# yuguangnudt/VEC_VAD

Hardware: AMD Instinct MI355X
Metric: spatio-temporal cubes/sec (train step) (higher is better)
Workload: dtype f32

## Files before the change

### vec_vad_amd/bank.py

```python
import ctypes as C
import math
import os
from collections import OrderedDict
from types import SimpleNamespace

import torch

from . import _lib as L

RAW_C, OF_C = 3, 2
HW0 = 32


def _ceil(a, b):
    return (a + b - 1) // b * b


def _pick_ksplit(groups, ntiles, ncu=256, epilogue=1.5, max_wg=1024):
    best, best_cost = 1, None
    for ks in range(1, ntiles + 1):
        if groups * ks > max_wg and ks > 1:
            break
        rounds = -(-groups * ks // ncu)
        cost = rounds * (-(-ntiles // ks) + epilogue)
        if best_cost is None or cost < best_cost - 1e-9:
            best, best_cost = ks, cost
    return best


class UnitSpec:

    def __init__(self, role, erase, tgt):
        self.role, self.erase, self.tgt = role, erase, tgt
        self.out_c = RAW_C if role == 'raw' else OF_C


class ConvLayer:
    def __init__(self, idx, H, cin, cout, mode, src, skip=None, up=None):
        self.idx, self.H, self.cin, self.cout, self.mode, self.src, self.skip, self.up = idx, H, cin, cout, mode, src, skip, up
        self.cinp = _ceil(cin, 16)


class BankLayout:

    def __init__(self, nf, in_ch):
        self.nf, self.in_ch = nf, in_ch
        c = nf
        Ls = [ConvLayer(0, 32, in_ch, nf, L.IN_CUBE, 'cube'), ConvLayer(1, 32, nf, nf, L.IN_ACT, 0)]
        H = 32
        for d in range(3):
            H //= 2
            Ls.append(ConvLayer(len(Ls), H, c, 2 * c, L.IN_POOL, len(Ls) - 1))
            Ls.append(ConvLayer(len(Ls), H, 2 * c, 2 * c, L.IN_ACT, len(Ls) - 1))
            c *= 2
        self.convT = []
        skips = [5, 3, 1]
        for u in range(3):
            self.convT.append((len(Ls) - 1, H, c, c // 2))
            H *= 2
            Ls.append(ConvLayer(len(Ls), H, c, c // 2, L.IN_CAT, None, skip=skips[u], up=u))
            Ls.append(ConvLayer(len(Ls), H, c // 2, c // 2, L.IN_ACT, len(Ls) - 1))
            c //= 2
        self.convs = Ls
        off = 0
        self.p = OrderedDict()
        for l in Ls:
            self.p['c%d.w' % l.idx] = (off, (l.cout, l.cin, 3, 3)); off += _ceil(l.cout * l.cin * 9, 4)
            self.p['c%d.b' % l.idx] = (off, (l.cout,)); off += l.cout
            self.p['c%d.g' % l.idx] = (off, (l.cout,)); off += l.cout
            self.p['c%d.beta' % l.idx] = (off, (l.cout,)); off += l.cout
        for u, (_, _, ci, co) in enumerate(self.convT):
            self.p['t%d.w' % u] = (off, (ci, co, 3, 3)); off += ci * co * 9
            self.p['t%d.b' % u] = (off, (co,)); off += co
        self.p['o.w'] = (off, (4, nf, 1, 1)); off += 4 * nf
        self.p['o.b'] = (off, (4,)); off += 4
        self.U = _ceil(off, 4)
        off = 0
        self.b = OrderedDict()
        for l in Ls:
            self.b['c%d.rm' % l.idx] = (off, (l.cout,)); off += l.cout
            self.b['c%d.rv' % l.idx] = (off, (l.cout,)); off += l.cout
        self.UB = _ceil(off, 4)
        off = 0
        self.pk = OrderedDict()
        for l in Ls:
            self.pk['c%d.f' % l.idx] = (off, 0, l.cin, l.cinp, l.cout, 'c%d.w' % l.idx); off += 9 * l.cinp * l.cout
            if l.idx > 0:
                self.pk['c%d.d' % l.idx] = (off, 1, l.cout, l.cout, l.cin, 'c%d.w' % l.idx); off += 9 * l.cout * l.cin
        for u, (_, _, ci, co) in enumerate(self.convT):
            self.pk['t%d.f' % u] = (off, 2, ci, ci, co, 't%d.w' % u); off += 9 * ci * co
            self.pk['t%d.d' % u] = (off, 3, co, co, ci, 't%d.w' % u); off += 9 * ci * co
        self.pkw = OrderedDict()
        for l in Ls:
            self.pkw['c%d.f' % l.idx] = (off, 0, l.cin, l.cinp, l.cout, 'c%d.w' % l.idx); off += 16 * l.cinp * l.cout
# ... 41 lines not shown
        for fn, args, label in self.calls:
            rc = fn(*args, stream)
            if rc:
                L.check(rc, label)


class UNetBank:
    def __init__(self, units, nf=32, tot_raw_num=5, tot_of_num=1, padding=False, active=None, device='cuda',
                 lambda_raw=1.0, lambda_of=1.0):
        self.lib = L.lib()
        self.ncu = int(self.lib.vv_num_cus())
        self.units = list(units)
        self.G = len(self.units)
        self.nf, self.tot_raw, self.tot_of, self.padding = nf, tot_raw_num, tot_of_num, padding
        if nf % 32:
            raise L.VecVadHipError('features_root must be a multiple of 32 for the MFMA tiles (got %d)' % nf)
        if nf not in (32, 64):
            raise L.VecVadHipError('features_root = %d: nf = 32 (the value of every shipped config.cfg) and nf = 64 (the default of '
                                   'SelfCompleteNet1raw1of, model/unet.py:563) are implemented -- the fused 1x1 output conv + loss '
                                   'kernels are instantiated for these two widths' % nf)
        self.in_ch = RAW_C * (tot_raw_num if padding else tot_raw_num - 1)
        self.lay = BankLayout(nf, self.in_ch)
        self.g0, self.Ga = active if active is not None else (0, self.G)
        self.lambda_raw, self.lambda_of = lambda_raw, lambda_of
        self.device = torch.device(device)
        self._alloc_state()
        self.ws = {}

    @property
    def adam_t(self):
        return self._adam_t

    @adam_t.setter
    def adam_t(self, t):
        self._adam_t = int(t)
        self._adam_t_dev.fill_(int(t))

    def _alloc_state(self):
        d, lay, G = self.device, self.lay, self.G
        nconv = len(lay.convs)

        def switch(name):
            v = os.environ.get(name, '1')
            if v not in ('0', '1'):
                raise ValueError('%s must be 0 or 1, got %r' % (name, v))
            return v == '1'

        def launch_set(name, default, words, names):
            v = os.environ.get(name, default).lower()
            if v.startswith('set:'):
                picked = frozenset(t for t in v[4:].split(',') if t)
                if not picked <= names:
                    raise ValueError('%s=%s: unknown entries %s' % (name, v, sorted(picked - names)))
                return picked
            if v not in words:
                raise ValueError('%s must be one of %s or set:..., got %r' % (name, ' / '.join(words), v))
            return '0' if v == 'off' else v

        self.precision = os.environ.get('VV_PRECISION', 'fp32').lower()
        if self.precision not in ('fp32', 'bf16'):
            raise ValueError("VV_PRECISION / [mi355x] precision must be 'fp32' or 'bf16', got %r" % self.precision)
        if self.nf != 32 and self.precision != 'fp32':
            raise L.VecVadHipError('mixed precision is implemented for features_root = 32 only')
        self.cflag = L.CONV_BF16 if self.precision == 'bf16' else 0
        self.dz16 = switch('VV_BF16_DZ') and bool(self.cflag)
        self.da16 = switch('VV_BF16_DA') and bool(self.cflag)
        self.y16 = switch('VV_BF16_Y') and self.dz16 and self.da16
        self.split_dcat = switch('VV_SPLIT_DCAT') and self.da16
        self.fflag = self.cflag | ((L.CONV_OUT_BF16 | L.CONV_ALLSRC_BF16) if self.y16 else 0)
        self.fuse_outconv = switch('VV_FUSE_OUTCONV')
        wino_env = switch('VV_WINOGRAD')
        self.wino = wino_env and not self.cflag
        self.wino_wgrad = switch('VV_WINOGRAD_WGRAD') and wino_env
        self.wgrad_flag = 256
        w44_words = ('0', 'off', '1', 'dgrad', 'all')
        w44_names = frozenset(['f%d' % i for i in range(nconv)] + ['d%d' % i for i in range(1, nconv)])
        self.w44_mode = launch_set('VV_WINO44', 'dgrad', w44_words, w44_names)
        self._w44_tables = {}
        self._w44_eval_used = set()
        self.w44_eval_mode = launch_set('VV_WINO44_EVAL', '1', w44_words, w44_names)
        self.fuse_bn_sums = switch('VV_FUSE_BN_SUMS')
        self.fuse_bn_sums_t = switch('VV_FUSE_BN_SUMS_T')
        fold = launch_set('VV_FUSE_BN_APPLY', '1', ('0', 'off', '1'), frozenset(str(i) for i in range(nconv)))
        self.fold_bn_apply = frozenset(int(t) for t in fold) if isinstance(fold, frozenset) else \
            frozenset() if fold == '0' else frozenset((0, 2, 4))
        self.group_reduce = switch('VV_GROUP_REDUCE')
        self.eval_fold = switch('VV_EVAL_FOLD') and not self.cflag

        self.params = torch.zeros(G, lay.U, device=d)
        self.bufs = torch.zeros(G, lay.UB, device=d)
        self.gb = [0, lay.p['c4.w'][0], lay.p['c8.w'][0], lay.U]
        self._gb_c = (C.c_int64 * len(self.gb))(*self.gb)
        self.grads = torch.zeros(G * lay.U, device=d)
        self.adam_m = None
        self.adam_v = None
        self._adam_t = 0
        self._adam_t_dev = torch.zeros(1, dtype=torch.long, device=d)
        self._adam_sc = torch.zeros(2, device=d)
        self.nbt = torch.zeros(G, len(lay.convs), dtype=torch.long, device=d)
        self.packed = torch.zeros(G, lay.UP, device=d)
        cin_p = lay.convs[0].cinp
        chmap = torch.full((G, cin_p), -1, dtype=torch.int32)
        oc = torch.zeros(G, dtype=torch.int32)
        tsrc = torch.zeros(G, dtype=torch.int32)
        tcoff = torch.zeros(G, dtype=torch.int32)
        for g, u in enumerate(self.units):
            if self.padding:
                for k in range(self.in_ch):
                    chmap[g, k] = -1 if u.erase * RAW_C <= k < (u.erase + 1) * RAW_C else k
            else:
                for k in range(self.in_ch):
                    chmap[g, k] = k if k < u.erase * RAW_C else k + RAW_C
            oc[g] = u.out_c
            tsrc[g] = 0 if u.role == 'raw' else 1
            tcoff[g] = u.tgt * (RAW_C if u.role == 'raw' else OF_C)
        self.chmap, self.oc, self.tsrc, self.tcoff = chmap.to(d), oc.to(d), tsrc.to(d), tcoff.to(d)
        direct = [(k, v) for k, v in lay.pk.items() if not (self.wino and k[0] == 'c')]
        ents = (L.PackEntry * len(direct))()
        mx = 0
        for i, (k, (off, mode, K, KP, N, src)) in enumerate(direct):
            ents[i] = L.PackEntry(lay.p[src][0], off, mode | (L.PACK_BF16 if self.cflag else 0), K, KP, N)
            mx = max(mx, 9 * KP * N)
        self.pack_table = torch.frombuffer(bytearray(bytes(ents)), dtype=torch.uint8).to(d)
        self.pack_n, self.pack_max = len(direct), mx
        head = lambda k: k[0] == 'c' and int(k[1:k.index('.')]) <= 1
        self.pack_head_n = sum(1 for k, _ in direct if head(k))
        assert all(head(k) for k, _ in direct[:self.pack_head_n])
        wents = (L.PackEntry * len(lay.pkw))()
        wmx = 0
        for i, (k, (off, mode, K, KP, N, src)) in enumerate(lay.pkw.items()):
            wents[i] = L.PackEntry(lay.p[src][0], off, mode, K, KP, N)
            wmx = max(wmx, KP * N)
        self.pack_table_w = torch.frombuffer(bytearray(bytes(wents)), dtype=torch.uint8).to(d)
        self.pack_w_n, self.pack_w_max = len(lay.pkw), wmx
        self.pack_w_head_n = sum(1 for k in lay.pkw if head(k))
        assert all(head(k) for k in list(lay.pkw)[:self.pack_w_head_n])
        self.eval_path = ('BatchNorm folded into filter + bias once per model state (vv_fold_bn), ReLU in the conv epilogue, plain loads'
                          if self.eval_fold else 'train-mode kernel family with running statistics')
        self.params_eval = self.packed_eval = None
        self._eval_key = None
        self._state_ver = 0
        fents = (L.FoldEntry * len(lay.convs))()
        for i, l in enumerate(lay.convs):
            fents[i] = L.FoldEntry(lay.p['c%d.w' % l.idx][0], lay.p['c%d.b' % l.idx][0], lay.p['c%d.g' % l.idx][0],
                                   lay.p['c%d.beta' % l.idx][0], lay.b['c%d.rm' % l.idx][0], lay.b['c%d.rv' % l.idx][0],
                                   l.cout, l.cin * 9)
        self.fold_table = torch.frombuffer(bytearray(bytes(fents)), dtype=torch.uint8).to(d)
        self.ab_ident = torch.stack([torch.ones(G, lay.cmax), torch.zeros(G, lay.cmax)]).to(d)

    def to(self, device):
        device = torch.device(device)
        if device == self.device:
            return self
        for n in ('params', 'bufs', 'grads', '_adam_t_dev', '_adam_sc', 'nbt', 'packed', 'chmap', 'oc', 'tsrc', 'tcoff', 'pack_table', 'pack_table_w', 'fold_table', 'ab_ident'):
            setattr(self, n, getattr(self, n).to(device))
        self._w44_tables, self._w44_eval_table = {}, None
        if self.adam_m is not None:
            self.adam_m, self.adam_v = self.adam_m.to(device), self.adam_v.to(device)
        self.device = device
        self.ws = {}
        self.params_eval = self.packed_eval = None
        self._eval_key = None
        return self

    def param_view(self, g, key):
        off, shape = self.lay.p[key]
        n = 1
        for s in shape:
# ... 377 lines not shown
        nf = self.nf
        f = lambda *s: torch.empty(*s, device=d, dtype=torch.float32)
        P = _Plan()
        pbase, kbase = self._p(self.params, g0 * U), self._p(self.packed, g0 * UP)
        abg = lay.cmax
        HWp = HW0 * HW0
        last = lay.convs[-1]
        self._alloc_outconv_bwd(ws, B)
        ws.D = {l.idx: f(Ga, B * l.H * l.H, l.cin) for l in lay.convs if l.idx > 0}

        def dcat_views(m):
            dcat = ws.D[m.idx]
            skipc = lay.convs[m.skip].cout
            if self.split_dcat and 2 * skipc == m.cin and skipc & (skipc - 1) == 0:
                plane = B * m.H * m.H * skipc * 2
                return (L.view(dcat, skipc, 0, dcat.stride(0)), L.view(dcat.data_ptr() + plane, skipc, 0, dcat.stride(0)), skipc)
            return (L.view(dcat, m.cin, 0, dcat.stride(0)), L.View(dcat.data_ptr(), dcat.stride(0), m.cin, skipc), 0)
        ws.DT = [f(Ga, B * H * H, ci) for (_, H, ci, co) in lay.convT]
        ws.dz2 = [f(Ga, B * HWp * nf), f(Ga, B * HWp * nf)]
        ws.dz = ws.dz2[0]
        ws.bnscr = f(Ga, 2 * lay.cmax)
        ws.bscr = f(Ga, (B * HWp + 1023) // 1024 * lay.cmax)
        ws.dstats = f(Ga, max(max(lib.vv_conv_ntiles2(B, l.H, l.H, L.CONV3, self.cflag), lib.vv_conv_ntiles(B, l.H, l.H),
                                  lib.vv_wino_ntiles(B, l.H)) * 2 * l.cin for l in lay.convs if l.mode == L.IN_CAT))

        t_of = {sidx: u for u, (sidx, _, _, _) in enumerate(lay.convT)}
        skip_of = {m.skip: m for m in lay.convs if m.mode == L.IN_CAT}
        pool_of = {m.src: m for m in lay.convs if m.mode == L.IN_POOL}
        act_of = {m.src: m for m in lay.convs if m.mode == L.IN_ACT}

        def dA_for(i):
            if i == last.idx:
                return L.view(ws.gA_last, nf, 0, ws.gA_last.stride(0)), None, 0
            if i in t_of:
                t = ws.DT[t_of[i]]
                return L.view(t, t.shape[2], 0, t.stride(0)), None, 0
            if i in skip_of:
                dp = ws.D[pool_of[i].idx] if i in pool_of else None
                return dcat_views(skip_of[i])[0], dp.data_ptr() if dp is not None else None, dp.stride(0) if dp is not None else 0
            dn = ws.D[i + 1]
            return L.view(dn, lay.convs[i + 1].cin, 0, dn.stride(0)), None, 0

        def wgrad(kind, H, cinp, cout, bf16_flags, wide):
            tiles = ((cinp + 31) // 32) * (cout // 32)
            nt = lib.vv_wgrad_ntiles(kind, B, H, H)
            ks = _pick_ksplit(Ga * tiles, nt, ncu=3 * self.ncu, max_wg=12 * self.ncu) if wide else \
                _pick_ksplit(Ga * tiles, nt, ncu=self.ncu, max_wg=4 * self.ncu)
            w = SimpleNamespace(bf16=False, ks=ks, kw=0)
            ntb, nblk, kw = C.c_int32(), C.c_int32(), C.c_int32()
            if self.cflag and lib.vv_wgrad_bf16_plan(kind | (bf16_flags << 8), B, H, H, cinp, cout,
                                                     C.byref(ntb), C.byref(nblk), C.byref(kw)):
                w = SimpleNamespace(bf16=True, ks=self._ks_bf16(Ga * nblk.value, ntb.value), kw=kw.value)
            w.nslab = w.ks * max(w.kw, 1)
            w.size = tiles * w.nslab * 9 * 1024
            return w

        rec = []
        for l in lay.convs:
            r = wgrad(L.CONV3, l.H, l.cinp, l.cout, (L.WGRAD_DY_BF16 | L.WGRAD_X_BF16) if self.y16 else 0,
                      self.wino_wgrad and not self.cflag)
            r.dA, r.dpool, r.dpg = dA_for(l.idx)
            r.dz16 = self.dz16 and r.bf16
            r.dflags = (self.cflag | ((L.CONV_ALLSRC_BF16 if self.y16 else L.CONV_SRC_BF16) if r.dz16 else 0) |
                        (L.CONV_OUT_BF16 if self.da16 else 0))
            r.dgrad = self._route(B, l, True, r.dflags) if l.idx > 0 else None
            r.partials, r.bn_sums_of = 0, None
            rec.append(r)
        trec = [wgrad(L.CONVT_FWD, H, ci, co, 0, False) for (_, H, ci, co) in lay.convT]
        for t in trec:
            t.bn_sums_of = None

        rec[last.idx].partials = L.BNBWD_PARTIALS_PER_CUBE
        for l in lay.convs:
            r, j = rec[l.idx], l.idx - 1
            if self.fuse_bn_sums and l.mode == L.IN_ACT and l.idx > 0 and l.src == j and j not in t_of and j not in skip_of \
                    and j not in pool_of and (self.wino or (self.y16 and r.bf16 and l.H == 32 and l.cin % 64 != 0)):
                r.bn_sums_of, rec[j].partials = j, r.dgrad[3]
        for u, (sidx, _, _, _) in enumerate(lay.convT):
            if self.fuse_bn_sums and self.fuse_bn_sums_t and not self.cflag and sidx != last.idx and sidx not in skip_of \
                    and sidx not in pool_of and sidx not in act_of:
                trec[u].bn_sums_of, rec[sidx].partials = sidx, L.BNBWD_PARTIALS_PER_TTILE

        for l, r in zip(lay.convs, rec):
            r.fold = (self.wino and self.wino_wgrad and l.idx in self.fold_bn_apply and l.idx != last.idx and l.cout <= 256
                      and r.dpool is None and (l.idx == 0 or (l.H in (16, 8) and r.dgrad[0] is not lib.vv_conv_wino44)))

        wtot = 0
        for w in rec + trec:
            w.woff, wtot = wtot, wtot + w.size
        ws.wpart = f(Ga, wtot)
        ws.bntab = {i: f(Ga, L.BNBWD_TAB_ROWS * lay.convs[i].cout) for i, r in enumerate(rec) if r.fold}
        wpg = ws.wpart.stride(0)
        pending = []

        def reduce_wgrad(key, kind, cin, cinp, cout, w, label, bucket_done, **kw_):
            gptr, gstride = self._g(key + '.w')
            if not self.group_reduce:
                P.add(lib.vv_wgrad_reduce, (kind, Ga, cin, cinp, cout, w.nslab, ws.wpart.data_ptr() + 4 * w.woff, wpg, gptr, gstride),
                      label, stream=1, **kw_)
                return
            pending.append((kind, cin, cinp, cout, w, gptr, gstride))
            if not bucket_done:
                return
            ents = (L.ReduceEntry * len(pending))()
            start = 0
            for n, (kind, cin, cinp, cout, w, gptr, gstride) in enumerate(pending):
                ents[n] = L.ReduceEntry(kind, cin, cout, cout // 32, w.nslab, start, w.woff, (gptr - self.grads.data_ptr()) // 4, gstride)
                start += ((cinp + 31) // 32) * (cout // 32) * 36
            tab = torch.frombuffer(bytearray(bytes(ents)), dtype=torch.uint8).to(d)
            P.keep.append(tab)
            P.add(lib.vv_wgrad_reduce_grouped, (tab.data_ptr(), len(pending), start, Ga, ws.wpart.data_ptr(), wpg, self.grads.data_ptr()),
                  label, stream=1, **kw_)
            del pending[:]

        def bn_sums(cp, j):
            yj = ws.y[j]
            cp.bn_z, cp.bn_z_gstride = yj.data_ptr(), yj.stride(0)
            cp.bn_a, cp.bn_b = self._p(ws.ab[0, j]), self._p(ws.ab[1, j])
            cp.bn_mean, cp.bn_invstd = self._p(ws.ab[2, j]), self._p(ws.ab[3, j])
            cp.bn_gstride, cp.bn_partial = abg, ws.bnpart.data_ptr()

        y = ws.y[last.idx]
        P.add(lib.vv_outconv_bwd, (Ga, B, HWp, nf, ws.dout4.data_ptr(), y.data_ptr(), y.stride(0), self._p(ws.ab[0, last.idx]),
                                   self._p(ws.ab[1, last.idx]), abg, pbase + 4 * lay.p['o.w'][0], U, ws.gA_last.data_ptr(),
                                   ws.gA_last.stride(0), ws.ocpart.data_ptr(),
                                   self._p(ws.ab[2, last.idx]), self._p(ws.ab[3, last.idx]), ws.bnpart.data_ptr(),
                                   (1 if self.da16 else 0) | (2 if self.y16 else 0)), 'outconv_bwd')
        assert self._g('o.w')[1] == self._g('o.b')[1]
        P.add(lib.vv_outconv_bwd_reduce, (Ga, nf, B, ws.ocpart.data_ptr(), self._p(self.oc, g0), self._g('o.w')[0],
                                          self._g('o.b')[0], self._g('o.w')[1]), 'outconv_bwd_reduce')

        order = [l.idx for l in reversed(lay.convs)]

        def conv_bwd(l):
            i, r = l.idx, rec[l.idx]
            y = ws.y[i]
            pos = order.index(i)
            dzb = ws.dz2[pos % 2]
            reuse_wait = ('wdone%d' % order[pos - 2],) if pos >= 2 and not r.fold else ()
            bp = L.BnBwdParams(Ga, B, l.H, l.H, l.cout,
                               (L.BNBWD_DZ_BF16 if r.dz16 else 0) | r.partials | (L.BNBWD_DA_BF16 if self.da16 else 0) |
                               (L.BNBWD_Y_BF16 if self.y16 else 0), y.data_ptr(), y.stride(0), self._p(ws.ab[0, i]), self._p(ws.ab[1, i]),
                               self._p(ws.ab[2, i]), self._p(ws.ab[3, i]), abg, r.dA, r.dpool, r.dpg, dzb.data_ptr(), dzb.stride(0),
                               ws.bnpart.data_ptr())
            P.keep.append(bp)
            if not r.partials:
                P.add(lib.vv_bn_bwd_reduce, (C.byref(bp),), 'bn_bwd_reduce%d' % i, wait=reuse_wait)
            if r.fold:
                tab = ws.bntab[i]
                P.add(lib.vv_bn_bwd_sums, (C.byref(bp), pbase + 4 * lay.p['c%d.g' % i][0], U, self._g('c%d.g' % i)[0],
                                           self._g('c%d.beta' % i)[0], self._g('c%d.g' % i)[1], tab.data_ptr(), tab.stride(0)),
                      'bn_bwd_sum%d' % i, record='dy%d' % i)
            else:
                P.add(lib.vv_bn_bwd_apply, (C.byref(bp), pbase + 4 * lay.p['c%d.g' % i][0], U, self._g('c%d.g' % i)[0],
                                            self._g('c%d.beta' % i)[0], self._g('c%d.g' % i)[1], ws.bnscr.data_ptr()), 'bn_bwd_apply%d' % i,
                      record='dy%d' % i, wait=reuse_wait if r.partials else ())
            if i > 0:
                Dl = ws.D[i]
                fn, panel = r.dgrad[:2]
                cp = L.ConvParams(L.CONV3, L.IN_PLAIN, Ga, B, l.H, l.H, l.cout, l.cout, l.cin,
                                  L.View(dzb.data_ptr(), dzb.stride(0), l.cout, 0), None, None, 0, L.NULL_VIEW, 0, r.dflags, None,
                                  kbase + 4 * panel, UP, None, 0, L.view(Dl, l.cin, 0, Dl.stride(0)),
                                  ws.dstats.data_ptr() if l.mode == L.IN_CAT else None)
                if r.fold:
                    cp.in_mode, cp.src0, cp.src1 = L.IN_BNBWD, r.dA, L.view(y, l.cout, 0, y.stride(0))
                    cp.a, cp.ab_gstride = ws.bntab[i].data_ptr(), ws.bntab[i].stride(0)
                if l.mode == L.IN_CAT:
                    v0, v1, osplit = dcat_views(l)
# ... 200 lines not shown
```

### vec_vad_amd/csrc/vv_wino44.hip

```cpp
#include <type_traits>
#include "vv_common.h"
namespace {

constexpr int W4N = 384;
constexpr int W4G = 2;
constexpr int W4T = 32;
constexpr int SB4_MASK = 0x386;
constexpr float PA = 0.75f, PB = 1.5f;
constexpr float PA2 = PA * PA, PB2 = PB * PB, PA3 = PA2 * PA, PB3 = PB2 * PB;
constexpr float PA2B2 = PA2 * PB2, PS2 = PA2 + PB2, PAB2 = PA * PB2, PA2B = PA2 * PB;

__device__ __forceinline__ void vv_lds_barrier4() {
  asm volatile("s_waitcnt lgkmcnt(0)" ::: "memory");
  __builtin_amdgcn_s_barrier();
  asm volatile("" ::: "memory");
}

template <int H_>
struct W4Geo {
  static constexpr int TPI = H_ / 4;
  static constexpr int TP = TPI * TPI;
  static constexpr int TPW = TP < W4T ? TP : W4T;
  static constexpr int NI = W4T / TPW;
  static constexpr int PARTS = TP / TPW;
  static constexpr int TROWS = TPW / TPI;
  static constexpr int HH = 4 * TROWS + 2, HW = H_ + 2;
  static constexpr int HWQ = (HW + 3) / 4;
  static constexpr int ROW = H_ == 32 ? 38 : (H_ == 16 ? 21 : (H_ == 8 ? 14 : 8));
  static constexpr int IMG = H_ == 32 ? HH * ROW : (H_ == 16 ? 400 : (H_ == 8 ? 146 : 49));
  static constexpr int PLANE = NI * IMG;
  static constexpr int tile_slot(const int l) {
    const int tim = l / TPW, rem = l % TPW;
    return tim * IMG + 4 * (rem / TPI) * ROW + rem % TPI;
  }
  static constexpr bool ok() {
    if (ROW < 4 * HWQ || IMG < HH * ROW) return false;
    for (int l0 = 0; l0 < 32; l0 += 16) {
      unsigned seen = 0;
      for (int l = l0; l < l0 + 16; ++l) {
        const unsigned bit = 1u << (tile_slot(l) & 15);
        if (seen & bit) return false;
        seen |= bit;
      }
    }
    return true;
  }
};
static_assert(W4Geo<32>::ok() && W4Geo<16>::ok() && W4Geo<8>::ok() && W4Geo<4>::ok(), "LDS image: bank conflicts or overlap");

template <int H_, bool NS>
__global__ void __launch_bounds__(W4N * W4G, 3)
wino44_conv_kernel(const vv_conv_params p, const int NT, const int NN, const int total, const int nper) {
  using G_ = W4Geo<H_>;
  constexpr int TPI = G_::TPI, TPW = G_::TPW, NI = G_::NI, PARTS = G_::PARTS, HH = G_::HH, HW = G_::HW, HWQ = G_::HWQ;
  constexpr int ROW = G_::ROW, IMG = G_::IMG, PLANE = G_::PLANE;
  constexpr int CK = 8, Q = 2;
  constexpr int HY0 = PARTS == 1 ? 1 : 0, HR = PARTS == 1 ? HH - 2 : HH;
  constexpr int NITEMS = NI * HR * H_ * Q;
  constexpr int STN = NS ? W4N * W4G : W4N;
  constexpr int NIT = (NITEMS + STN - 1) / STN;
  constexpr int HALO8 = 4 * PLANE;
  constexpr int EX8 = 6 * 8 * 64 * 2;
  constexpr int L8 = HALO8 > EX8 ? HALO8 : EX8;
  __shared__ v2f lds_all[W4G][L8 + 6 * 32 + 256];
  const int wv = __builtin_amdgcn_readfirstlane((int)(threadIdx.x >> 6));
  const int sg = wv / 6;
  v2f* const lds8 = lds_all[sg];
  float* lds = reinterpret_cast<float*>(lds8);
  v2f* const halo = NS ? lds_all[0] : lds8;

  int w = vv_xcd_remap(blockIdx.x, nper);
  if (w >= total) return;
  int nn, pt, g;
  bool live = true;
  if constexpr (NS) {
    const int NNW = NN / W4G;
    nn = (w % NNW) * W4G + sg; w /= NNW;
    pt = w % NT;
    g = w / NT;
  } else {
    nn = w % NN; w /= NN;
    const int NTP = (NT + W4G - 1) / W4G;
    const int pt_ = (w % NTP) * W4G + sg;
    live = pt_ < NT;
    pt = live ? pt_ : NT - 1;
    g = w / NTP;
  }

  const int tid = threadIdx.x - sg * W4N, lane = tid & 63, half = lane >> 5, l31 = lane & 31;
  const int stid = NS ? (int)threadIdx.x : tid;
  const int xi = wv - sg * 6;
  const int img0 = (pt / PARTS) * NI, part = pt % PARTS;
  const int y0 = part * (4 * G_::TROWS) - 1;
  const VVSrc s = vv_make_src(p, g, H_, H_);
  const int Cout = p.Cout, CinP = p.CinP, KQ = CinP >> 3;
  const int co0 = nn * 32;
  const float* __restrict__ wg = p.w + (int64_t)g * p.w_gstride;

  unsigned valid = 0;
  unsigned itm[NIT];
  const int tile = (img0 * H_ + y0) * H_ - 1;
  const int q4 = (stid % Q) * 4;
  for (int hp = stid; hp < NI * HH * HW; hp += STN) {
    const int hx = hp % HW, t = hp / HW;
    const int hy = t % HH, im = t / HH;
    if (hx == 0 || hx == HW - 1 || hy < HY0 || hy >= HY0 + HR) {
      const int sl = im * IMG + hy * ROW + (hx & 3) * HWQ + (hx >> 2);
#pragma unroll
      for (int pl = 0; pl < 4; ++pl) halo[pl * PLANE + sl] = (v2f){0.f, 0.f};
    }
  }
#pragma unroll
  for (int k = 0; k < NIT; ++k) {
    const int it = stid + k * STN;
    const int q = it % Q, hp = it / Q;
    const int hx = hp % H_ + 1, t = hp / H_;
    const int hy = t % HR + HY0, im = t / HR;
    const bool inr = NITEMS % STN == 0 || it < NITEMS;
    const int y = y0 + hy;
    const bool ok = inr && (unsigned)y < (unsigned)H_ && (img0 + im) < s.B;
    valid |= ok ? (1u << k) : 0u;
    const int pixv = (im * H_ + hy) * H_ + hx;
    const int sl = inr ? q * 2 * PLANE + im * IMG + hy * ROW + (hx & 3) * HWQ + (hx >> 2) : 0xFFFF;
    itm[k] = ((unsigned)sl << 16) | (unsigned)pixv;
  }
  static_assert((NI * H_ + HH) * H_ + HW < 65536 && 4 * PLANE < 65535, "packed item word");
  const __amdgpu_buffer_rsrc_t rsW = __builtin_amdgcn_make_buffer_rsrc(const_cast<float*>(wg), 0, 0x7FFFFFFF, 0x00020000);
  const unsigned bvo = (unsigned)(half * Cout + co0 + l31) * 8u;
  const int bsub = 2 * Cout * 8;
  const int bnu = KQ * 2 * bsub;
  const int bxi = xi * 6 * bnu;
  const int nact = s.mode == VV_IN_ACT ? CinP : (s.mode == VV_IN_CAT ? s.csplit : 0);
  float4* const ab4 = reinterpret_cast<float4*>((NS ? lds_all[0] : lds8) + L8 + 6 * 32);
  for (int i = stid; i < (nact >> 2); i += STN) {
    ab4[i] = *reinterpret_cast<const float4*>(s.a + 4 * i);
    ab4[(CinP >> 2) + i] = *reinterpret_cast<const float4*>(s.b + 4 * i);
  }
  float4 r[NIT];
  auto issue = [&](const int c0) {
    const bool second = __builtin_amdgcn_readfirstlane((int)((s.mode == VV_IN_CAT) && c0 >= s.csplit)) != 0;
    const float* base = second ? s.p1 + s.co1 : s.p0 + s.co0;
    const int cs = second ? s.cs1 : s.cs0;
    const __amdgpu_buffer_rsrc_t rs = __builtin_amdgcn_make_buffer_rsrc(const_cast<float*>(base), 0, 0x7FFFFFFF, 0x00020000);
    const int soff = (second ? c0 - s.csplit : c0) * 4;
#pragma unroll
    for (int k = 0; k < NIT; ++k) {
      const unsigned vo_ = ((unsigned)((tile + (int)(itm[k] & 0xFFFFu)) * cs + q4) * 4u) |
                           ((((valid >> k) & 1u) ^ 1u) << 31);
      const v4f v = __builtin_amdgcn_raw_buffer_load_b128(rs, vo_, soff, 0);
      r[k] = make_float4(v.x, v.y, v.z, v.w);
    }
  };
  auto commit = [&](const int c0) {
    const bool act = c0 < nact;
    float4 sa = make_float4(1.f, 1.f, 1.f, 1.f), sb = make_float4(0.f, 0.f, 0.f, 0.f);
    if (act) {
      sa = ab4[(c0 + q4) >> 2];
      sb = ab4[(CinP >> 2) + ((c0 + q4) >> 2)];
    }
#pragma unroll
    for (int k = 0; k < NIT; ++k) {
      const int sl = (int)(itm[k] >> 16);
      if (NITEMS % STN == 0 || k < NIT - 1 || sl != 0xFFFF) {
        float4 v = r[k];
        if (act) {
          const float4 a = vv_act4(v, sa, sb);
          const bool vk = (valid >> k) & 1u;
          v = make_float4(vk ? a.x : v.x, vk ? a.y : v.y, vk ? a.z : v.z, vk ? a.w : v.w);
        }
        halo[sl] = (v2f){v.x, v.y};
        halo[sl + PLANE] = (v2f){v.z, v.w};
      }
    }
  };
  v2f u[6];
  auto load_u = [&](const int step, const int n) -> v2f {
    return __builtin_bit_cast(v2f, __builtin_amdgcn_raw_buffer_load_b64(rsW, bvo, bxi + n * bnu + step * bsub, 0));
  };

  const int pbase = half * 2 * PLANE + G_::tile_slot(l31);

  v16f acc[6];
  const int nsteps = 2 * KQ;
  auto substep = [&](const auto XI_, const int step, const auto SUB_, const auto first, const auto LAST_) {
    constexpr int XI = decltype(XI_)::value, sub = decltype(SUB_)::value;
    constexpr bool LAST = decltype(LAST_)::value;
    const int nxt = step + 1;
    int pb = pbase;
    asm volatile("" : "+v"(pb));
    const v2f* const pp = halo + pb + sub * PLANE;
    v2f R[6];
#pragma unroll
    for (int b = 0; b < 6; ++b) {
      const int o = (b & 3) * HWQ + (b >> 2);
      if constexpr (XI == 0) {
        R[b] = PA2B2 * pp[o] - PS2 * pp[2 * ROW + o] + pp[4 * ROW + o];
      } else if constexpr (XI == 5) {
        R[b] = PA2B2 * pp[ROW + o] - PS2 * pp[3 * ROW + o] + pp[5 * ROW + o];
      } else {
        const v2f d1 = pp[ROW + o], d2 = pp[2 * ROW + o], d3 = pp[3 * ROW + o], d4 = pp[4 * ROW + o];
        if constexpr (XI == 1) R[b] = (d4 - PB2 * d2) + (PA * d3 - PAB2 * d1);
        if constexpr (XI == 2) R[b] = (d4 - PB2 * d2) - (PA * d3 - PAB2 * d1);
        if constexpr (XI == 3) R[b] = (d4 - PA2 * d2) + (PB * d3 - PA2B * d1);
        if constexpr (XI == 4) R[b] = (d4 - PA2 * d2) - (PB * d3 - PA2B * d1);
      }
    }
    v2f V[6];
    {
      const v2f pq = R[4] - PB2 * R[2], qq = PA * R[3] - PAB2 * R[1], rr = R[4] - PA2 * R[2], ss = PB * R[3] - PA2B * R[1];
      V[0] = PA2B2 * R[0] - PS2 * R[2] + R[4];
      V[1] = pq + qq;
      V[2] = pq - qq;
      V[3] = rr + ss;
      V[4] = rr - ss;
      V[5] = PA2B2 * R[1] - PS2 * R[3] + R[5];
    }
    __builtin_amdgcn_sched_barrier(SB4_MASK);
#define W4_X(n)                                                                                        \
    if constexpr (decltype(first)::value) {                                                             \
      const v16f z = {0.f, 0.f, 0.f, 0.f, 0.f, 0.f, 0.f, 0.f, 0.f, 0.f, 0.f, 0.f, 0.f, 0.f, 0.f, 0.f};   \
      acc[n] = __builtin_amdgcn_mfma_f32_32x32x2f32(V[n].x, u[n].x, z, 0, 0, 0);                         \
    } else {                                                                                            \
      acc[n] = __builtin_amdgcn_mfma_f32_32x32x2f32(V[n].x, u[n].x, acc[n], 0, 0, 0);                    \
    }
#define W4_Y(n) acc[n] = __builtin_amdgcn_mfma_f32_32x32x2f32(V[n].y, u[n].y, acc[n], 0, 0, 0);
#pragma unroll
    for (int n = 0; n < 6; ++n) {
      W4_X(n)
      W4_Y(n)
      __builtin_amdgcn_sched_barrier(SB4_MASK);
      if constexpr (!LAST) u[n] = load_u(nxt, n);
      __builtin_amdgcn_sched_barrier(SB4_MASK);
    }
#undef W4_X
#undef W4_Y
  };
// ... 163 lines not shown
    float* sp = lds + L8 * 2;
    if (half == 0) {
      sp[xi * 32 + l31] = s1;
      sp[(6 + xi) * 32 + l31] = s2;
    }
    __syncthreads();
    if (tid < 32 && live) {
      float t1 = 0.f, t2 = 0.f;
#pragma unroll
      for (int k = 0; k < 6; ++k) {
        t1 += sp[k * 32 + tid];
        t2 += sp[(6 + k) * 32 + tid];
      }
      float* st = sout + ((int64_t)(g * NT + pt) * 2) * Cout + co0 + tid;
      st[0] = t1;
      st[Cout] = t2;
    }
  }
}

__global__ void __launch_bounds__(VV_WG)
wino44_pack_kernel(const vv_pack_entry* __restrict__ table, const float* __restrict__ params, const int64_t params_gstride,
                   float* __restrict__ packed, const int64_t packed_gstride) {
  __shared__ float ex[36][256];
  const vv_pack_entry e = table[blockIdx.y];
  const int g = blockIdx.z;
  const float* src = params + (int64_t)g * params_gstride + e.src_off;
  float* dst = packed + (int64_t)g * packed_gstride + e.dst_off;
  const int KQ = e.KP >> 3, NB = e.N >> 5;
  const int t = threadIdx.x, kl = t & 7, nl = t >> 3;
  for (int blk = blockIdx.x; blk < KQ * NB; blk += gridDim.x) {
    const int kq = blk / NB, nb = blk % NB;
    const int k = kq * 8 + kl, n = nb * 32 + nl;
    float gk[3][3];
#pragma unroll
    for (int a = 0; a < 3; ++a)
#pragma unroll
      for (int b = 0; b < 3; ++b) {
        float v = 0.f;
        if (k < e.K) v = e.mode == 0 ? src[((int64_t)n * e.K + k) * 9 + a * 3 + b]
                                     : src[((int64_t)k * e.N + n) * 9 + (2 - a) * 3 + (2 - b)];
        gk[a][b] = v;
      }
    auto grow = [](const int i, const double x, const double y, const double z) -> double {
      constexpr double a = PA, b = PB, a2 = a * a, b2 = b * b;
      constexpr double n0 = a2 * b2, na = 2.0 * a2 * (a2 - b2), nb = 2.0 * b2 * (b2 - a2);
      switch (i) {
        case 0: return x / n0;
        case 1: return (x + a * y + a2 * z) / na;
        case 2: return (x - a * y + a2 * z) / na;
        case 3: return (x + b * y + b2 * z) / nb;
        case 4: return (x - b * y + b2 * z) / nb;
        default: return z;
      }
    };
    double rr[6][3];
#pragma unroll
    for (int i = 0; i < 6; ++i)
#pragma unroll
      for (int b = 0; b < 3; ++b) rr[i][b] = grow(i, gk[0][b], gk[1][b], gk[2][b]);
    const int hf = kl >> 2, sub = (kl & 3) >> 1, j = kl & 1;
    const int slot = (sub * 2 + hf) * 64 + nl * 2 + j;
    __syncthreads();
#pragma unroll
    for (int xi = 0; xi < 6; ++xi)
#pragma unroll
      for (int nu = 0; nu < 6; ++nu) ex[xi * 6 + nu][slot] = (float)grow(nu, rr[xi][0], rr[xi][1], rr[xi][2]);
    __syncthreads();
    const int sh = t >> 6, rem = t & 63;
#pragma unroll
    for (int xn = 0; xn < 36; ++xn)
      dst[((((int64_t)xn * KQ + kq) * 4 + sh) * e.N + nb * 32) * 2 + rem] = ex[xn][t];
  }
}

template <int H_>
int launch_wino44(const vv_conv_params* p, hipStream_t st) {
  using G_ = W4Geo<H_>;
  const int NT = ((p->B + G_::NI - 1) / G_::NI) * G_::PARTS;
  const int NN = p->Cout / 32;
  if (NN % W4G == 0) {
    const int total = p->G * (NN / W4G) * NT;
    const int nper = (total + 7) / 8;
    VV_LAUNCH((wino44_conv_kernel<H_, true>), dim3(nper * 8), dim3(W4N * W4G), 0, st, *p, NT, NN, total, nper);
  } else {
    const int total = p->G * NN * ((NT + W4G - 1) / W4G);
    const int nper = (total + 7) / 8;
    VV_LAUNCH((wino44_conv_kernel<H_, false>), dim3(nper * 8), dim3(W4N * W4G), 0, st, *p, NT, NN, total, nper);
  }
  VV_CHECK_LAUNCH();
  return VV_OK;
}

}

extern "C" int vv_wino44_ntiles(int32_t B, int32_t H) {
  switch (H) {
    case 32: return ((B + W4Geo<32>::NI - 1) / W4Geo<32>::NI) * W4Geo<32>::PARTS;
    case 16: return ((B + W4Geo<16>::NI - 1) / W4Geo<16>::NI) * W4Geo<16>::PARTS;
    case 8: return ((B + W4Geo<8>::NI - 1) / W4Geo<8>::NI) * W4Geo<8>::PARTS;
    case 4: return ((B + W4Geo<4>::NI - 1) / W4Geo<4>::NI) * W4Geo<4>::PARTS;
  }
  return -1;
}

extern "C" int vv_conv_wino44(const vv_conv_params* p, vv_stream stream) {
  if (!p || !p->src0.ptr || !p->w || !p->out.ptr) return VV_ERR_BAD_ARG;
  if (p->G <= 0 || p->B <= 0 || p->kind != VV_CONV3 || p->H != p->W) return VV_ERR_BAD_ARG;
  if (p->Cout % 32 || p->CinP % 8 || p->CinP > 256) return VV_ERR_UNSUPPORTED;
  if (p->out1.ptr) return VV_ERR_UNSUPPORTED;
  if (p->bn_partial && (p->stats || !p->bn_z || !p->bn_a || !p->bn_b || !p->bn_mean || !p->bn_invstd)) return VV_ERR_BAD_ARG;
  {
    const int64_t px = (int64_t)p->B * p->H * p->W * 4;
    const int64_t cs = p->out.cstride > p->Cout ? p->out.cstride : p->Cout;
    if (px * cs >= (1ll << 31)) return VV_ERR_UNSUPPORTED;
  }
  if (p->in_mode != VV_IN_PLAIN && p->in_mode != VV_IN_ACT && p->in_mode != VV_IN_CAT)
    return VV_ERR_UNSUPPORTED;
  if (p->in_mode == VV_IN_CAT && p->csplit % 8) return VV_ERR_UNSUPPORTED;
  hipStream_t st = (hipStream_t)stream;
  switch (p->H) {
    case 32: return launch_wino44<32>(p, st);
    case 16: return launch_wino44<16>(p, st);
    case 8: return launch_wino44<8>(p, st);
    case 4: return launch_wino44<4>(p, st);
  }
  return VV_ERR_UNSUPPORTED;
}

extern "C" int vv_pack_wino44(const vv_pack_entry* table_dev, int32_t nentries, int32_t G, const float* params,
                              int64_t params_gstride, float* packed, int64_t packed_gstride, int32_t max_kn,
                              vv_stream stream) {
  if (!table_dev || !params || !packed || nentries <= 0) return VV_ERR_BAD_ARG;
  int bx = (max_kn + VV_WG - 1) / VV_WG;
  if (bx > 64) bx = 64;
  if (bx < 1) bx = 1;
  VV_LAUNCH(wino44_pack_kernel, dim3(bx, nentries, G), dim3(VV_WG), 0, (hipStream_t)stream, table_dev, params, params_gstride,
            packed, packed_gstride);
  VV_CHECK_LAUNCH();
  return VV_OK;
}
```

Measured before the change: 29180.

## Fold BN-backward apply into Winograd F(4,3) dgrad input staging for 16/8 layers

Adds a BNBWD input mode to the wino44 conv kernel. It loads both the upstream gradient and the saved activation through buffer loads, applies the batch-norm backward affine using a per-channel table staged in LDS, and writes the result into the halo image. The fold policy now covers wino44 dgrad layers at H=16/8 whose channel count is a multiple of 64, and layer 11 joins the default fold set. This removes a separate BN-apply pass and its intermediate tensor round trip, at the cost of a larger LDS footprint that may lower occupancy, and twice the global loads per input tile.

```diff
diff --git a/vec_vad_amd/bank.py b/vec_vad_amd/bank.py
--- a/vec_vad_amd/bank.py
+++ b/vec_vad_amd/bank.py
@@ -10,6 +10,7 @@
 
 RAW_C, OF_C = 3, 2
 HW0 = 32
+FOLD_DEFAULT = frozenset((0, 2, 4, 11))
 
 
 def _ceil(a, b):
@@ -217,8 +218,9 @@
         self.fuse_bn_sums = switch('VV_FUSE_BN_SUMS')
         self.fuse_bn_sums_t = switch('VV_FUSE_BN_SUMS_T')
         fold = launch_set('VV_FUSE_BN_APPLY', '1', ('0', 'off', '1'), frozenset(str(i) for i in range(nconv)))
+        self.fold_bn_probe = isinstance(fold, frozenset)
         self.fold_bn_apply = frozenset(int(t) for t in fold) if isinstance(fold, frozenset) else \
-            frozenset() if fold == '0' else frozenset((0, 2, 4))
+            frozenset() if fold == '0' else FOLD_DEFAULT
         self.group_reduce = switch('VV_GROUP_REDUCE')
         self.eval_fold = switch('VV_EVAL_FOLD') and not self.cflag
 
@@ -762,8 +764,10 @@
                 trec[u].bn_sums_of, rec[sidx].partials = sidx, L.BNBWD_PARTIALS_PER_TTILE
 
         for l, r in zip(lay.convs, rec):
+            on44 = l.idx > 0 and r.dgrad[0] is lib.vv_conv_wino44
             r.fold = (self.wino and self.wino_wgrad and l.idx in self.fold_bn_apply and l.idx != last.idx and l.cout <= 256
-                      and r.dpool is None and (l.idx == 0 or (l.H in (16, 8) and r.dgrad[0] is not lib.vv_conv_wino44)))
+                      and r.dpool is None and (l.idx == 0 or (l.H in (16, 8) and (not on44 or l.cin % 64 == 0))
+                                               or (l.H == 32 and self.fold_bn_probe and not on44)))
 
         wtot = 0
         for w in rec + trec:
diff --git a/vec_vad_amd/csrc/vv_wino44.hip b/vec_vad_amd/csrc/vv_wino44.hip
--- a/vec_vad_amd/csrc/vv_wino44.hip
+++ b/vec_vad_amd/csrc/vv_wino44.hip
@@ -48,7 +48,7 @@
 };
 static_assert(W4Geo<32>::ok() && W4Geo<16>::ok() && W4Geo<8>::ok() && W4Geo<4>::ok(), "LDS image: bank conflicts or overlap");
 
-template <int H_, bool NS>
+template <int H_, bool NS, bool BNB>
 __global__ void __launch_bounds__(W4N * W4G, 3)
 wino44_conv_kernel(const vv_conv_params p, const int NT, const int NN, const int total, const int nper) {
   using G_ = W4Geo<H_>;
@@ -62,7 +62,9 @@
   constexpr int HALO8 = 4 * PLANE;
   constexpr int EX8 = 6 * 8 * 64 * 2;
   constexpr int L8 = HALO8 > EX8 ? HALO8 : EX8;
-  __shared__ v2f lds_all[W4G][L8 + 6 * 32 + 256];
+  constexpr int TAB8 = BNB ? VV_BNBWD_TAB_ROWS * 256 / 2 : 256;
+  static_assert(!BNB || NS, "VV_IN_BNBWD: the table lives in the shared halo image's group");
+  __shared__ v2f lds_all[W4G][L8 + 6 * 32 + TAB8];
   const int wv = __builtin_amdgcn_readfirstlane((int)(threadIdx.x >> 6));
   const int sg = wv / 6;
   v2f* const lds8 = lds_all[sg];
@@ -136,8 +138,26 @@
     ab4[i] = *reinterpret_cast<const float4*>(s.a + 4 * i);
     ab4[(CinP >> 2) + i] = *reinterpret_cast<const float4*>(s.b + 4 * i);
   }
+  const float* const bnt = reinterpret_cast<const float*>(ab4);
+  if constexpr (BNB) {
+    for (int i = stid; i < ((VV_BNBWD_TAB_ROWS * CinP) >> 2); i += STN) ab4[i] = *reinterpret_cast<const float4*>(s.a + 4 * i);
+  }
   float4 r[NIT];
+  float4 rz[BNB ? NIT : 1];
   auto issue = [&](const int c0) {
+    if constexpr (BNB) {
+      const __amdgpu_buffer_rsrc_t rsA = __builtin_amdgcn_make_buffer_rsrc(const_cast<float*>(s.p0 + s.co0), 0, 0x7FFFFFFF, 0x00020000);
+      const __amdgpu_buffer_rsrc_t rsY = __builtin_amdgcn_make_buffer_rsrc(const_cast<float*>(s.p1 + s.co1), 0, 0x7FFFFFFF, 0x00020000);
+#pragma unroll
+      for (int k = 0; k < NIT; ++k) {
+        const unsigned px = (unsigned)(tile + (int)(itm[k] & 0xFFFFu)), inv = (((valid >> k) & 1u) ^ 1u) << 31;
+        const v4f v = __builtin_amdgcn_raw_buffer_load_b128(rsA, ((px * (unsigned)s.cs0 + q4) * 4u) | inv, c0 * 4, 0);
+        r[k] = make_float4(v.x, v.y, v.z, v.w);
+        const v4f z = __builtin_amdgcn_raw_buffer_load_b128(rsY, ((px * (unsigned)s.cs1 + q4) * 4u) | inv, c0 * 4, 0);
+        rz[k] = make_float4(z.x, z.y, z.z, z.w);
+      }
+      return;
+    }
     const bool second = __builtin_amdgcn_readfirstlane((int)((s.mode == VV_IN_CAT) && c0 >= s.csplit)) != 0;
     const float* base = second ? s.p1 + s.co1 : s.p0 + s.co0;
     const int cs = second ? s.cs1 : s.cs0;
@@ -152,6 +172,22 @@
     }
   };
   auto commit = [&](const int c0) {
+    if constexpr (BNB) {
+      const VVBnBwd4 kc = vv_bnbwd_consts(bnt, CinP, c0 + q4);
+#pragma unroll
+      for (int k = 0; k < NIT; ++k) {
+        const int sl = (int)(itm[k] >> 16);
+        if (NITEMS % STN == 0 || k < NIT - 1 || sl != 0xFFFF) {
+          float4 v = r[k];
+          const float4 d = vv_bnbwd4(v, rz[k], kc);
+          const bool vk = (valid >> k) & 1u;
+          v = make_float4(vk ? d.x : v.x, vk ? d.y : v.y, vk ? d.z : v.z, vk ? d.w : v.w);
+          halo[sl] = (v2f){v.x, v.y};
+          halo[sl + PLANE] = (v2f){v.z, v.w};
+        }
+      }
+      return;
+    }
     const bool act = c0 < nact;
     float4 sa = make_float4(1.f, 1.f, 1.f, 1.f), sb = make_float4(0.f, 0.f, 0.f, 0.f);
     if (act) {
@@ -481,11 +517,19 @@
   if (NN % W4G == 0) {
     const int total = p->G * (NN / W4G) * NT;
     const int nper = (total + 7) / 8;
-    VV_LAUNCH((wino44_conv_kernel<H_, true>), dim3(nper * 8), dim3(W4N * W4G), 0, st, *p, NT, NN, total, nper);
+    if (p->in_mode == VV_IN_BNBWD) {
+      if constexpr (H_ == 16 || H_ == 8)
+        VV_LAUNCH((wino44_conv_kernel<H_, true, true>), dim3(nper * 8), dim3(W4N * W4G), 0, st, *p, NT, NN, total, nper);
+      else
+        return VV_ERR_UNSUPPORTED;
+    } else
+      VV_LAUNCH((wino44_conv_kernel<H_, true, false>), dim3(nper * 8), dim3(W4N * W4G), 0, st, *p, NT, NN, total, nper);
+  } else if (p->in_mode == VV_IN_BNBWD) {
+    return VV_ERR_UNSUPPORTED;
   } else {
     const int total = p->G * NN * ((NT + W4G - 1) / W4G);
     const int nper = (total + 7) / 8;
-    VV_LAUNCH((wino44_conv_kernel<H_, false>), dim3(nper * 8), dim3(W4N * W4G), 0, st, *p, NT, NN, total, nper);
+    VV_LAUNCH((wino44_conv_kernel<H_, false, false>), dim3(nper * 8), dim3(W4N * W4G), 0, st, *p, NT, NN, total, nper);
   }
   VV_CHECK_LAUNCH();
   return VV_OK;
@@ -514,7 +558,12 @@
     const int64_t cs = p->out.cstride > p->Cout ? p->out.cstride : p->Cout;
     if (px * cs >= (1ll << 31)) return VV_ERR_UNSUPPORTED;
   }
-  if (p->in_mode != VV_IN_PLAIN && p->in_mode != VV_IN_ACT && p->in_mode != VV_IN_CAT)
+  if (p->in_mode == VV_IN_BNBWD) {
+    if (!p->src1.ptr || !p->a || p->Cin != p->CinP || (p->pad0 & (VV_CONV_BF16 | VV_CONV_RELU))) return VV_ERR_BAD_ARG;
+    if ((p->H != 16 && p->H != 8) || (p->Cout / 32) % W4G) return VV_ERR_UNSUPPORTED;
+    const int64_t scs = p->src1.cstride > p->src0.cstride ? p->src1.cstride : p->src0.cstride;
+    if ((int64_t)p->B * p->H * p->W * scs * 4 >= (1ll << 31)) return VV_ERR_UNSUPPORTED;
+  } else if (p->in_mode != VV_IN_PLAIN && p->in_mode != VV_IN_ACT && p->in_mode != VV_IN_CAT)
     return VV_ERR_UNSUPPORTED;
   if (p->in_mode == VV_IN_CAT && p->csplit % 8) return VV_ERR_UNSUPPORTED;
   hipStream_t st = (hipStream_t)stream;
```

Result: no change. 29200 (median of 3 runs) (+0.1%).
